# pierric/smart-chess-rust

Hardware: AMD Instinct MI355X
Metric: MCTS simulations/sec (whole node), self-play rollout=180, at 1/2/4/8 MI355X (higher is better)
Workload: dtype bf16

## Files before the change

smart-chess-rust_amd/csrc/nn_tower32.hpp:

```cpp
#pragma once
#include <type_traits>

#include "nn_kernels.hpp"

namespace scnn {

typedef __attribute__((ext_vector_type(16))) float f32x16;
typedef __attribute__((ext_vector_type(8))) int i32x8;

struct PrecBF16 {
    static constexpr bool FP8 = false;
    static constexpr int EB = 2;
    static constexpr int KS = 16;
    static constexpr int FB = 16;
    typedef bf16x8 frag;
};
struct PrecFP8 {
    static constexpr bool FP8 = true;
    static constexpr int EB = 1;
    static constexpr int KS = 64;
    static constexpr int FB = 32;
    typedef i32x8 frag;
};
template <class P>
// ... 109 lines not shown
    static_assert(TAPS % TPI == 0 && SPG % RS == 0 && PD < SPG, "bad ring / tap-group geometry");
    static_assert(SPG % AB == 0 && AD <= SPG, "bad image buffer geometry");
    const __amdgpu_buffer_rsrc_t rsrc = __builtin_amdgcn_make_buffer_rsrc(
        const_cast<bf16_t*>(Wp) + (size_t)wave_u * CT * (TB / 2), 0, 0x7fffffff, 0x00020000);
    const int voff = lane * 16;
    auto toffb = [](int t) { return (TAPS == 9) ? ((((t * 11) >> 5) - 1) * 10 + (t - 3 * ((t * 11) >> 5)) - 1) * PSB : 0; };
    frag xq[AB][2];
    int wcur = 0;
    int pc[TPI][2];
#pragma unroll
    for (int tl = 0; tl < TPI; tl++)
#pragma unroll
        for (int pt = 0; pt < 2; pt++) pc[tl][pt] = xoff + px[pt] + toffb(tl);
    if (!PRE) {
#pragma unroll
        for (int st = 0; st < PD; st++)
#pragma unroll
            for (int ct = 0; ct < CT; ct++) bq[st][ct] = wload_p<P>(rsrc, voff, ct, st * SBB);
    }
#pragma unroll
    for (int v = 0; v < AD; v++)
#pragma unroll
        for (int pt = 0; pt < 2; pt++) xq[v][pt] = lds_frag_p<P>(pc[v / KPT][pt] + (v % KPT) * KSB);
#pragma unroll 1
    for (int j = 0; j < NG; j++) {
        const int tn = (j + 1 == NG) ? 0 : j + 1;
        const int wnext = (j == NG - 1) ? next_first : tn * (SPG * SBB);
        int pn[TPI][2];
#pragma unroll
        for (int tl = 0; tl < TPI; tl++)
#pragma unroll
            for (int pt = 0; pt < 2; pt++) pn[tl][pt] = xoff + px[pt] + toffb(tn * TPI + tl);
#pragma unroll
        for (int u = 0; u < SPG; u++) {
            const int slot = u % RS;
#pragma unroll
            for (int ct = 0; ct < CT; ct++)
                bq[(slot + PD) % RS][ct] = (u + PD < SPG) ? wload_p<P>(rsrc, voff, ct, wcur + (u + PD) * SBB)
                                                          : wload_p<P>(rsrc, voff, ct, wnext + (u + PD - SPG) * SBB);
#pragma unroll
            for (int pt = 0; pt < 2; pt++) {
                const int v = u + AD;
                xq[v % AB][pt] = (v < SPG) ? lds_frag_p<P>(pc[v / KPT][pt] + (v % KPT) * KSB)
                                           : lds_frag_p<P>(pn[(v - SPG) / KPT][pt] + ((v - SPG) % KPT) * KSB);
            }
#pragma unroll
            for (int ct = 0; ct < CT; ct++)
#pragma unroll
                for (int pt = 0; pt < 2; pt++)
                    acc[ct][pt] = mma_p<P>(bq[slot][ct], xq[u % AB][pt], acc[ct][pt], sa[ct]);
#pragma unroll
            for (int m = 0; m < 2 * CT; m++) {
                __builtin_amdgcn_sched_group_barrier(0x008, 1, 0);
                if (P::FP8) {
                    __builtin_amdgcn_sched_group_barrier(0x100, CT == 1 ? 2 : 1, 0);
                    __builtin_amdgcn_sched_group_barrier(0x020, 1, 0);
                } else if (CT == 1) {
                    __builtin_amdgcn_sched_group_barrier(0x100, 1, 0);
                    if (m == 0) __builtin_amdgcn_sched_group_barrier(0x020, 1, 0);
                } else {
                    if ((m & 1) == 0)
                        __builtin_amdgcn_sched_group_barrier(0x100, 1, 0);
                    else
                        __builtin_amdgcn_sched_group_barrier(0x020, 1, 0);
                }
            }
            __builtin_amdgcn_sched_barrier(0);
        }
        wcur = wnext;
#pragma unroll
        for (int tl = 0; tl < TPI; tl++)
#pragma unroll
            for (int pt = 0; pt < 2; pt++) pc[tl][pt] = pn[tl][pt];
    }
}

struct LnStat {
    float rstd[2], nm[2];
};
template <int CT>
__device__ inline void ln_reduce(const f32x16 (&acc)[CT][2], LnStat& L, int count, int wave, int lane, float* s_stat2,
                                 int& parity, int& bad) {
    float2* st = reinterpret_cast<float2*>(s_stat2) + (parity & 1) * 256;
    parity ^= 1;
    const int i = lane & 31;
    float s[2], q[2];
#pragma unroll
    for (int pt = 0; pt < 2; pt++) {
        f32x2 a2 = {0.f, 0.f}, b2 = {0.f, 0.f};
#pragma unroll
        for (int ct = 0; ct < CT; ct++)
#pragma unroll
            for (int r = 0; r < 16; r += 2) {
                const f32x2 v = pair(acc[ct][pt], r);
                a2 += v;
                b2 = v * v + b2;
            }
        s[pt] = a2.x + a2.y;
        q[pt] = b2.x + b2.y;
    }
    {
        const auto rs = __builtin_amdgcn_permlane32_swap(__float_as_uint(s[0]), __float_as_uint(s[1]), false, false);
        const auto rq = __builtin_amdgcn_permlane32_swap(__float_as_uint(q[0]), __float_as_uint(q[1]), false, false);
        st[wave * 64 + lane] = make_float2(__uint_as_float(rs[0]) + __uint_as_float(rs[1]), __uint_as_float(rq[0]) + __uint_as_float(rq[1]));
    }
    __syncthreads();
    const float inv = 1.0f / (float)count;
#pragma unroll
    for (int pt = 0; pt < 2; pt++) {
        const int gp = pt * 32 + i;
        float2 a0 = st[gp], a1 = st[64 + gp], a2 = st[128 + gp], a3 = st[192 + gp];
        float S = (a0.x + a1.x) + (a2.x + a3.x);
        float Q = (a0.y + a1.y) + (a2.y + a3.y);
        float mean = S * inv;
        float var = Q * inv - mean * mean;
        bad |= (var != var) ? 1 : 0;
        var = fmaxf(var, 0.f);
        L.rstd[pt] = __frsqrt_rn(var + 1e-6f);
        L.nm[pt] = -mean * L.rstd[pt];
    }
}
template <int CT>
__device__ __forceinline__ void ln_apply(f32x16 (&acc)[CT][2], const LnStat& L, const ChP<CT>& G, const ChP<CT>& E, bool relu) {
#pragma unroll
    for (int pt = 0; pt < 2; pt++)
#pragma unroll
        for (int ct = 0; ct < CT; ct++)
#pragma unroll
            for (int r = 0; r < 16; r += 2) {
                const f32x2 t = pair(acc[ct][pt], r) * splat(L.rstd[pt]) + splat(L.nm[pt]);
                const f32x2 y = t * pair(G.v[ct][r >> 2], r & 3) + pair(E.v[ct][r >> 2], r & 3);
                acc[ct][pt][r] = relu ? fmaxf(y.x, 0.f) : y.x;
                acc[ct][pt][r + 1] = relu ? fmaxf(y.y, 0.f) : y.y;
            }
}
template <class P, int CT>
__device__ __forceinline__ void ln_apply_relu_store(const f32x16 (&acc)[CT][2], const LnStat& L, const ChP<CT>& G, const ChP<CT>& E,
                                                    const int (&pixbase)[2], int wave, int h) {
#pragma unroll
    for (int ct = 0; ct < CT; ct++)
#pragma unroll
        for (int pt = 0; pt < 2; pt++)
#pragma unroll
            for (int g = 0; g < 4; g++) {
                f32x2 y[2];
#pragma unroll
                for (int hf = 0; hf < 2; hf++) {
                    const f32x2 t = pair(acc[ct][pt], 4 * g + 2 * hf) * splat(L.rstd[pt]) + splat(L.nm[pt]);
                    y[hf] = t * pair(G.v[ct][g], 2 * hf) + pair(E.v[ct][g], 2 * hf);
                }
                store4<P, true>(pixbase[pt], chan32<CT>(wave, ct, g, h), y[0], y[1]);
            }
}
template <int CT>
__device__ inline void layernorm32(f32x16 (&acc)[CT][2], const ChP<CT>& G, const ChP<CT>& E, int count, bool relu, int wave,
                                   int lane, float* s_stat2, int& parity, int& bad) {
    LnStat L;
    ln_reduce<CT>(acc, L, count, wave, lane, s_stat2, parity, bad);
    ln_apply<CT>(acc, L, G, E, relu);
}

template <class P, int CT>
__device__ inline void store_image32(const f32x16 (&acc)[CT][2], const int (&pixbase)[2], int wave, int h) {
#pragma unroll
    for (int ct = 0; ct < CT; ct++)
#pragma unroll
        for (int pt = 0; pt < 2; pt++)
#pragma unroll
            for (int g = 0; g < 4; g++)
                store4<P, false>(pixbase[pt], chan32<CT>(wave, ct, g, h), pair(acc[ct][pt], 4 * g), pair(acc[ct][pt], 4 * g + 2));
}

template <int CTRL>
__device__ __forceinline__ float dpp_mov(float x) { return dpp_f<CTRL>(x); }
template <int LVL>
__device__ __forceinline__ float pool_xchg(float x) {
    if constexpr (LVL == 1) return dpp_mov<0x140>(x);
    else if constexpr (LVL == 2) return dpp_mov<0x141>(x);
    else if constexpr (LVL == 3) return dpp_mov<0x4E>(x);
    else return dpp_mov<0xB1>(x);
}
template <int NV, int W, int LVL>
__device__ __forceinline__ void pool_level(float (&v)[NV], int lane) {
    if constexpr (LVL < 5) {
        if constexpr (W >= 1) {
            if constexpr (LVL == 0) {
#pragma unroll
                for (int t = 0; t < W; t++) {
                    const auto r = __builtin_amdgcn_permlane16_swap(__float_as_uint(v[t]), __float_as_uint(v[t + W]), false, false);
                    v[t] = __uint_as_float(r[0]) + __uint_as_float(r[1]);
                }
            } else {
                const bool hi = (lane & (16 >> LVL)) != 0;
#pragma unroll
                for (int t = 0; t < W; t++) {
                    float send = hi ? v[t] : v[t + W], keep = hi ? v[t + W] : v[t];
                    v[t] = keep + pool_xchg<LVL>(send);
                }
            }
            pool_level<NV, W / 2, LVL + 1>(v, lane);
        } else {
            v[0] += pool_xchg<LVL>(v[0]);
            pool_level<NV, 0, LVL + 1>(v, lane);
        }
    }
}

template <class P, int CT, int TILES, int RS>
__device__ __forceinline__ void ring_fill(typename P::frag (&bq)[RS][CT], const bf16_t* __restrict__ Wp, int wave_u, int lane) {
    constexpr int TB = 64 * P::FB;
    const __amdgpu_buffer_rsrc_t rsrc = __builtin_amdgcn_make_buffer_rsrc(
        const_cast<bf16_t*>(Wp) + (size_t)wave_u * CT * (TB / 2), 0, 0x7fffffff, 0x00020000);
#pragma unroll
    for (int st = 0; st < RS - 1; st++)
#pragma unroll
        for (int ct = 0; ct < CT; ct++) bq[st][ct] = wload_p<P>(rsrc, lane * 16, ct, st * TILES * TB);
}
template <class P, int CT>
__device__ __forceinline__ void scale_load(int (&sa)[CT], const NetDev& net, int conv_idx, int wave, int lane) {
#pragma unroll
    for (int ct = 0; ct < CT; ct++)
        sa[ct] = P::FP8 ? __builtin_bit_cast(int, net.wf[net.f_scales + (size_t)((conv_idx * 8 + wave * CT + ct) * 64 + lane)]) : 127;
}

template <class P, int C>
struct TowerLds {
    static constexpr int IMG_BYTES = (100 * pix_stride<P>(C) > 4864 * 4) ? 100 * pix_stride<P>(C) : 4864 * 4;
    static constexpr int HIMG_BYTES = 64 * pix_stride<P>(HEAD);
    static constexpr int HIMG = IMG_BYTES;
    static constexpr int STAT = HIMG + HIMG_BYTES;
    static constexpr int VEC = STAT + 4096;
    static constexpr int SCL = VEC + 3072;
    static constexpr int RED = SCL + 1024;
    static constexpr int PAR = RED + 64;
    static constexpr int TOTAL = PAR + 15 * C * 2;
    static_assert(4864 * 4 <= IMG_BYTES, "policy logits (and the softmax pass that reads 19 x 256 of them) must fit in the image area");
    static_assert(IMG_BYTES % 16 == 0 && HIMG_BYTES % 16 == 0, "LDS regions must stay 16-byte aligned");
    static_assert(6 * HEAD * 4 + 3 * POL_PAD * 4 <= TOTAL - VEC, "head parameters must fit in the staging area");
};
static_assert(TowerLds<PrecBF16, 128>::TOTAL == 73088 && TowerLds<PrecBF16, 256>::TOTAL == 102528, "bf16 tower LDS");
static_assert(TowerLds<PrecFP8, 128>::TOTAL == 48960 && TowerLds<PrecFP8, 256>::TOTAL == 60544, "fp8 tower LDS");

struct NoPre {
    __device__ __forceinline__ bool operator()(int) const { return true; }
};
struct Fc1Hand {
    typedef __attribute__((ext_vector_type(4))) unsigned int u32x4;
    Fc1W w;
    uint32_t early;
    int have_a;
    u32x4 a[8];
};
struct NoHand {};
template <class P, int C, int RS, int TPI, int AB = SC_T32_AB, class Pre = NoPre, class Hand = NoHand>
__device__ __forceinline__ bool tower_body(const TowerArgs& A, const int pos, const int8_t* planes_lds, Pre pre, Hand& fhr) {
    constexpr bool FUSED = !std::is_same<Pre, NoPre>::value;
    constexpr bool HAND = std::is_same<Hand, Fc1Hand>::value;
    Hand* const fh = &fhr;
    typedef typename P::frag frag;
    constexpr int CT = C / 128;
    constexpr int TILES = C / 32;
    constexpr int PSB = pix_stride<P>(C);
    constexpr int HPSB = pix_stride<P>(HEAD);
    constexpr int EB = P::EB;
    constexpr int HRS = P::FP8 ? C / 64 : 8, HAB = P::FP8 ? 2 : SC_T32_AB;
    constexpr int H2RS = P::FP8 ? HEAD / 64 : 16, H2AB = P::FP8 ? 2 : SC_T32_AB;
    constexpr int NTW = C / 64;
    typedef TowerLds<P, C> Lds;
    unsigned char* smem = g_smem;
    float* s_stat = reinterpret_cast<float*>(smem + Lds::STAT);
    float* s_scl = reinterpret_cast<float*>(smem + Lds::SCL);
    float* s_red = reinterpret_cast<float*>(smem + Lds::RED);
    bf16_t* s_xb = reinterpret_cast<bf16_t*>(smem + Lds::VEC);
    float* s_z = reinterpret_cast<float*>(smem);

    const int tid = threadIdx.x, lane = tid & 63;
    const int wave = __builtin_amdgcn_readfirstlane(tid >> 6);
    const int i32 = lane & 31, h = lane >> 5;
    const NetDev& net = A.net;
    const int bp[2] = {gpix2board(0, i32), gpix2board(1, i32)};
    const int pixbase[2] = {hidx(bp[0]) * PSB, hidx(bp[1]) * PSB};
    const int px[2] = {pixbase[0] + h * P::FB, pixbase[1] + h * P::FB};

    frag ring[RS][CT];
    int sa[CT], san[CT];
    scale_load<P, CT>(sa, net, 0, wave, lane);
    scale_load<P, CT>(san, net, net.n_blocks > 0 ? 1 : 1 + 2 * net.n_blocks, wave, lane);
    ChP<CT> Bn;
    const int p_in = tid >> 2, q_in = tid & 3;
    uint32_t win[7];
    if (!FUSED && !planes_lds) {
        const uint32_t* src = reinterpret_cast<const uint32_t*>(A.boards + (size_t)pos * 7168 + p_in * 112 + q_in * 28);
#pragma unroll
        for (int k = 0; k < 7; k++) win[k] = src[k];
    }
    static_assert(C <= 256, "one parameter vector per thread");
    f32x4 spv = f32x4{0.f, 0.f, 0.f, 0.f};
    if (tid < 3 * C / 4) spv = *reinterpret_cast<const f32x4*>(net.wf + net.f_stem + tid * 4);
    else if (tid < C) spv = *reinterpret_cast<const f32x4*>(net.wf + net.f_blocks + (tid - 3 * C / 4) * 4);
    if (!FUSED || wave != 0) ring_fill<P, CT, TILES, RS>(ring, net.wb + net.o_stem, wave, lane);
    __builtin_amdgcn_sched_barrier(0);
    if constexpr (FUSED) {
        __shared__ int s_go;
        if (wave <= 1) {
            const bool go = pre(wave);
            if (wave == 0 && lane == 0) s_go = go ? 1 : 0;
            if (wave == 0) ring_fill<P, CT, TILES, RS>(ring, net.wb + net.o_stem, wave, lane);
        } else {
            uint4* z = reinterpret_cast<uint4*>(smem);
            for (int k = tid - 128; k < 100 * PSB / 16; k += 128) z[k] = make_uint4(0, 0, 0, 0);
        }
        __syncthreads();
        if (!s_go) return false;
    } else {
        uint4* z = reinterpret_cast<uint4*>(smem);
        for (int k = tid; k < 100 * PSB / 16; k += 256) z[k] = make_uint4(0, 0, 0, 0);
        __syncthreads();
    }
    if (FUSED || planes_lds) {
        const uint32_t* src = reinterpret_cast<const uint32_t*>(planes_lds + p_in * 112 + q_in * 28);
#pragma unroll
        for (int k = 0; k < 7; k++) win[k] = src[k];
    }
    {
        uint32_t* dst = reinterpret_cast<uint32_t*>(smem + hidx(p_in) * PSB + q_in * 28 * EB);
#pragma unroll
        for (int k = 0; k < 7; k++) {
            const uint32_t w = win[k];
            float v[4];
#pragma unroll
            for (int b = 0; b < 4; b++) v[b] = (float)(int8_t)((w >> (8 * b)) & 0xff);
            if constexpr (P::FP8) {
                dst[k] = pk_fp8x4(v[0], v[1], v[2], v[3]);
            } else {
                dst[2 * k] = pk_bf16(f32x2{v[0], v[1]});
                dst[2 * k + 1] = pk_bf16(f32x2{v[2], v[3]});
            }
        }
        if (tid < C) *reinterpret_cast<f32x4*>(g_smem + Lds::PAR + tid * 16) = spv;
    }
    __syncthreads();

    f32x16 acc[CT][2];
    int ln_parity = 0;
    int bad = 0;
    f32x16 res[CT][2];
    auto store_res = [&]() {
#pragma unroll
        for (int ct = 0; ct < CT; ct++)
#pragma unroll
            for (int pt = 0; pt < 2; pt++) res[ct][pt] = acc[ct][pt];
    };
    auto dump = [&](int stage) {
        if constexpr (FUSED) return;
        if (A.dbg && A.dbg_stage == stage) {
#pragma unroll
            for (int ct = 0; ct < CT; ct++)
#pragma unroll
                for (int pt = 0; pt < 2; pt++)
#pragma unroll
                    for (int r = 0; r < 16; r++)
                        A.dbg[((size_t)pos * 64 + bp[pt]) * C + chan32<CT>(wave, ct, r >> 2, h) + (r & 3)] = acc[ct][pt][r];
        }
    };

    {
        ch_load_lds<CT>(Bn, Lds::PAR, wave, h);
        acc_init<CT>(acc, Bn);
        const bf16_t* w0 = net.wb + net.o_stem;
        conv_mma32<P, 128, 9, CT, TILES, PSB, RS, TPI, true, AB>(0, w0, wave, lane, px, acc, ring, (int)((net.wb + net.o_blocks) - w0) * 2, sa);
        ChP<CT> G, E;
        ch_load_lds<CT>(G, Lds::PAR + C * 4, wave, h);
        ch_load_lds<CT>(E, Lds::PAR + 2 * C * 4, wave, h);
        ch_load_lds<CT>(Bn, Lds::PAR + 3 * C * 4, wave, h);
        layernorm32<CT>(acc, G, E, C, true, wave, lane, s_stat, ln_parity, bad);
    }
    store_res();
    store_image32<P, CT>(acc, pixbase, wave, h);
    __syncthreads();
    dump(0);
    const int head_conv0 = 1 + 2 * net.n_blocks;

#pragma unroll 1
    for (int b = 0; b < net.n_blocks; b++) {
        const bf16_t* wb = net.wb + net.o_blocks + (size_t)b * net.blk_stride_b;
        const float* wf = net.wf + net.f_blocks + (size_t)b * net.blk_stride_f;
        constexpr int NT1 = C / 32;
        constexpr int NTW1 = NT1 / 4;
        constexpr int PAR_V4 = 15 * C / 8;
        constexpr int NPV = (PAR_V4 + 255) / 256;
        constexpr int P_G1 = Lds::PAR, P_E1 = Lds::PAR + 4 * C, P_B2 = Lds::PAR + 8 * C, P_G2 = Lds::PAR + 12 * C, P_E2 = Lds::PAR + 16 * C;
        constexpr int P_SB1 = Lds::PAR + 20 * C, P_SB2 = Lds::PAR + 22 * C, P_BN = Lds::PAR + 26 * C;
        f32x4 pv[NPV];
#pragma unroll
        for (int k = 0; k < NPV; k++)
            if (tid + 256 * k < PAR_V4) pv[k] = *reinterpret_cast<const f32x4*>(wf + C + (size_t)(tid + 256 * k) * 4);
        __builtin_amdgcn_sched_barrier(0);
        acc_init<CT>(acc, Bn);
#pragma unroll
        for (int ct = 0; ct < CT; ct++) sa[ct] = san[ct];
        scale_load<P, CT>(san, net, 2 + 2 * b, wave, lane);
        conv_mma32<P, C, 9, CT, TILES, PSB, RS, TPI, true, AB>(0, wb, wave, lane, px, acc, ring, 9 * C * C * EB, sa);
#pragma unroll
        for (int k = 0; k < NPV; k++)
            if (tid + 256 * k < PAR_V4) *reinterpret_cast<f32x4*>(g_smem + Lds::PAR + (tid + 256 * k) * 16) = pv[k];
        {
            LnStat L;
            ln_reduce<CT>(acc, L, C, wave, lane, s_stat, ln_parity, bad);
            ChP<CT> G, E;
            ch_load_lds<CT>(G, P_G1, wave, h);
            ch_load_lds<CT>(E, P_E1, wave, h);
            ln_apply_relu_store<P, CT>(acc, L, G, E, pixbase, wave, h);
        }
        ch_load_lds<CT>(Bn, P_B2, wave, h);
        __syncthreads();
        acc_init<CT>(acc, Bn);
        {
            const int nxt = (b + 1 < net.n_blocks) ? (int)(net.blk_stride_b * 2 - (size_t)9 * C * C * EB) : 0;
#pragma unroll
            for (int ct = 0; ct < CT; ct++) sa[ct] = san[ct];
            scale_load<P, CT>(san, net, b + 1 < net.n_blocks ? 3 + 2 * b : head_conv0, wave, lane);
            conv_mma32<P, C, 9, CT, TILES, PSB, RS, TPI, true, AB>(0, wb + (size_t)9 * C * C * EB / 2, wave, lane, px, acc, ring, nxt, sa);
        }
        VecW<C, NTW1> w1;
        VecW<C / 2, NTW> w2;
        vec_w_load<C, NTW1, NT1>(w1, wb + (size_t)9 * C * C * EB, wave * NTW1, lane);
        vec_w_load<C / 2, NTW, C / 16>(w2, wb + (size_t)9 * C * C * EB + (size_t)C * (C / 2), wave * NTW, lane);
        __builtin_amdgcn_sched_barrier(0);
        {
            LnStat L;
            ln_reduce<CT>(acc, L, C, wave, lane, s_stat, ln_parity, bad);
            ChP<CT> G, E;
            ch_load_lds<CT>(G, P_G2, wave, h);
            ch_load_lds<CT>(E, P_E2, wave, h);
            ln_apply<CT>(acc, L, G, E, false);
        }
        {
            constexpr int NV = 16 * CT;
            float v[NV];
#pragma unroll
            for (int ct = 0; ct < CT; ct++)
#pragma unroll
                for (int r = 0; r < 16; r += 2) {
                    const f32x2 t = pair(acc[ct][0], r) + pair(acc[ct][1], r);
                    v[ct * 16 + r] = t.x;
                    v[ct * 16 + r + 1] = t.y;
                }
            pool_level<NV, NV / 2, 0>(v, lane);
            const int idx = (NV == 32) ? i32 : (i32 >> 1);
            s_xb[chan32<CT>(wave, idx >> 4, (idx & 15) >> 2, h) + (idx & 3)] = f2bf(v[0] * (1.0f / 64.0f));
        }
        float sb1[NTW1], sb2[NTW];
#pragma unroll
        for (int k = 0; k < NTW1; k++) sb1[k] = *reinterpret_cast<const float*>(g_smem + P_SB1 + (wave * (16 * NTW1) + (lane & 15) * NTW1 + k) * 4);
#pragma unroll
        for (int k = 0; k < NTW; k++) sb2[k] = *reinterpret_cast<const float*>(g_smem + P_SB2 + (chan0<NTW>(wave, lane) + k) * 4);
        __syncthreads();
        bf16_t* s_hid = s_xb + 256;
        {
            f32x4 hh[NTW1];
#pragma unroll
            for (int k = 0; k < NTW1; k++) hh[k] = f32x4{0.f, 0.f, 0.f, 0.f};
            vec_mma<C, NTW1>(s_xb, w1, lane, hh);
            if (lane < 16) {
#pragma unroll
                for (int k = 0; k < NTW1; k++) {
                    const int j = wave * (16 * NTW1) + (lane & 15) * NTW1 + k;
                    float t = hh[k][0] + sb1[k];
                    s_hid[j] = f2bf(fmaxf(t, 0.f));
                }
            }
        }
        __syncthreads();
        {
            f32x4 sc[NTW];
#pragma unroll
            for (int k = 0; k < NTW; k++) sc[k] = f32x4{0.f, 0.f, 0.f, 0.f};
            vec_mma<C / 2, NTW>(s_hid, w2, lane, sc);
            if (lane < 16) {
                const int c0 = chan0<NTW>(wave, lane);
#pragma unroll
                for (int k = 0; k < NTW; k++)
                    s_scl[c0 + k] = __builtin_amdgcn_rcpf(1.0f + __expf(-(sc[k][0] + sb2[k])));
            }
        }
#pragma unroll
        for (int ct = 0; ct < CT; ct++)
#pragma unroll
            for (int g = 0; g < 4; g++) {
                const int ch = chan32<CT>(wave, ct, g, h);
                const f32x4 sv = *reinterpret_cast<const f32x4*>(s_scl + ch);
#pragma unroll
                for (int pt = 0; pt < 2; pt++) {
                    const f32x4 rv = f32x4{res[ct][pt][4 * g], res[ct][pt][4 * g + 1], res[ct][pt][4 * g + 2], res[ct][pt][4 * g + 3]};
#pragma unroll
                    for (int k = 0; k < 4; k += 2) {
                        const f32x2 y = pair(acc[ct][pt], 4 * g + k) * pair(sv, k) + pair(rv, k);
                        acc[ct][pt][4 * g + k] = fmaxf(y.x, 0.f);
                        acc[ct][pt][4 * g + k + 1] = fmaxf(y.y, 0.f);
                    }
                }
            }
        store_res();
        store_image32<P, CT>(acc, pixbase, wave, h);
        ch_load_lds<CT>(Bn, P_BN, wave, h);
        __syncthreads();
        dump(b + 1);
    }
    dump(1000);

    const int gpb[2] = {i32 * HPSB, (32 + i32) * HPSB};
    constexpr int HP_V = Lds::VEC, HP_P1 = Lds::VEC + 3 * HEAD * 4, HP_P2 = Lds::VEC + 6 * HEAD * 4;
    f32x4 hpv[2];
#pragma unroll
    for (int k = 0; k < 2; k++)
        if (tid + 256 * k < 480) hpv[k] = *reinterpret_cast<const f32x4*>(net.wf + net.f_vhead + (size_t)(tid + 256 * k) * 4);
    __builtin_amdgcn_sched_barrier(0);
    frag hr[HRS][2];
    frag hr2[H2RS][1];
    int sh[2], sh2[1];
    scale_load<P, 2>(sh, net, head_conv0, wave, lane);
    {
        f32x16 hv[2][2];
#pragma unroll
        for (int ct = 0; ct < 2; ct++)
#pragma unroll
            for (int pt = 0; pt < 2; pt++)
#pragma unroll
                for (int r = 0; r < 16; r++) hv[ct][pt][r] = 0.f;
        conv_mma32<P, C, 1, 2, 8, PSB, HRS, 1, false, HAB>(0, net.wb + net.o_vconv, wave, lane, px, hv, hr,
                                                           (int)((net.wb + net.o_pconv1) - (net.wb + net.o_vconv)) * 2, sh);
        scale_load<P, 2>(sh, net, head_conv0 + 1, wave, lane);
        scale_load<P, 1>(sh2, net, head_conv0 + 2, wave, lane);
#pragma unroll
        for (int k = 0; k < 2; k++)
            if (tid + 256 * k < 480) *reinterpret_cast<f32x4*>(g_smem + Lds::VEC + (tid + 256 * k) * 16) = hpv[k];
        __builtin_amdgcn_sched_barrier(0);
        __syncthreads();
        ChP<2> Bv, G, E;
        ch_load_lds<2>(Bv, HP_V, wave, h);
#pragma unroll
        for (int ct = 0; ct < 2; ct++)
#pragma unroll
            for (int pt = 0; pt < 2; pt++)
#pragma unroll
                for (int r = 0; r < 16; r++) hv[ct][pt][r] += Bv.v[ct][r >> 2][r & 3];
        LnStat L;
        int badv = bad;
        ln_reduce<2>(hv, L, HEAD, wave, lane, s_stat, ln_parity, badv);
        ch_load_lds<2>(G, HP_V + HEAD * 4, wave, h);
        ch_load_lds<2>(E, HP_V + 2 * HEAD * 4, wave, h);
        ln_apply<2>(hv, L, G, E, true);
        const __amdgpu_buffer_rsrc_t hrs = __builtin_amdgcn_make_buffer_rsrc(A.hval + (size_t)pos * (64 * HEAD), 0, 0x7fffffff, 0x00020000);
        const bool wt = HAND && A.fc1_arrive;
#pragma unroll
        for (int ct = 0; ct < 2; ct++)
#pragma unroll
            for (int pt = 0; pt < 2; pt++) {
                const int off = (((wave * 2 + ct) * 2 + pt) * 64 + lane) * 32;
#pragma unroll
                for (int q = 0; q < 2; q++) {
                    typedef __attribute__((ext_vector_type(4))) unsigned int u32x4;
                    u32x4 v = {pk_bf16(pair(hv[ct][pt], 8 * q)), pk_bf16(pair(hv[ct][pt], 8 * q + 2)), pk_bf16(pair(hv[ct][pt], 8 * q + 4)),
                               pk_bf16(pair(hv[ct][pt], 8 * q + 6))};
                    if (badv) v = u32x4{0x7fc07fc0u, 0x7fc07fc0u, 0x7fc07fc0u, 0x7fc07fc0u};
                    if (wt) __builtin_amdgcn_raw_buffer_store_b128(v, hrs, off + 16 * q, 0, AUX_SC1);
                    else __builtin_amdgcn_raw_buffer_store_b128(v, hrs, off + 16 * q, 0, 0);
                }
            }
    }
    {
        ChP<2> Bv, G, E;
        ch_load_lds<2>(Bv, HP_P1, wave, h);
        f32x16 hp[2][2];
        acc_init<2>(hp, Bv);
        conv_mma32<P, C, 1, 2, 8, PSB, HRS, 1, true, HAB>(0, net.wb + net.o_pconv1, wave, lane, px, hp, hr, 0, sh);
        if (HAND && A.fc1_arrive) asm volatile("s_waitcnt vmcnt(0)" ::: "memory");
        ring_fill<P, 1, 4, H2RS>(hr2, net.wb + net.o_pconv2, wave, lane);
        __builtin_amdgcn_sched_barrier(0);
        LnStat L;
        ln_reduce<2>(hp, L, HEAD, wave, lane, s_stat, ln_parity, bad);
        if (HAND && A.fc1_arrive && tid == 0)
            __hip_atomic_fetch_add(A.fc1_arrive + (pos >> 6) * 32, 1u, __ATOMIC_RELAXED, __HIP_MEMORY_SCOPE_AGENT);
        ch_load_lds<2>(G, HP_P1 + HEAD * 4, wave, h);
        ch_load_lds<2>(E, HP_P1 + 2 * HEAD * 4, wave, h);
        ln_apply<2>(hp, L, G, E, false);
        const int xb[2] = {Lds::HIMG + gpb[0], Lds::HIMG + gpb[1]};
        store_image32<P, 2>(hp, xb, wave, h);
    }
    __syncthreads();
    {
        ChP<1> Bv, G, E;
        ch_load_lds<1>(Bv, HP_P2, wave, h);
        f32x16 z[1][2];
        acc_init<1>(z, Bv);
        const int pxh[2] = {gpb[0] + h * P::FB, gpb[1] + h * P::FB};
        conv_mma32<P, HEAD, 1, 1, 4, HPSB, H2RS, 1, true, H2AB>(Lds::HIMG, net.wb + net.o_pconv2, wave, lane, pxh, z, hr2, 0, sh2);
        uint32_t first = 0;
        if (HAND && A.fc1_arrive && tid == 0 && !A.fc1_acquire)
            first = __hip_atomic_load(A.fc1_arrive + (pos >> 6) * 32, __ATOMIC_RELAXED, __HIP_MEMORY_SCOPE_AGENT);
        LnStat L;
        ln_reduce<1>(z, L, 73, wave, lane, s_stat, ln_parity, bad);
        ch_load_lds<1>(G, HP_P2 + POL_PAD * 4, wave, h);
        ch_load_lds<1>(E, HP_P2 + 2 * POL_PAD * 4, wave, h);
        ln_apply<1>(z, L, G, E, false);
        __syncthreads();
#pragma unroll
        for (int pt = 0; pt < 2; pt++)
#pragma unroll
            for (int r = 0; r < 16; r++) {
                const int ch = chan32<1>(wave, 0, r >> 2, h) + (r & 3);
                if (ch < 73) s_z[ch * 64 + bp[pt]] = z[0][pt][r];
            }
// ... 59 lines not shown
```

smart-chess-rust_amd/csrc/search_select.hpp:

```cpp
#pragma once
#include <type_traits>
#include <hip/hip_runtime.h>

#include "mcts_types.hpp"
#include "position_chain.hpp"

namespace sc {

using scw::dpp_i, scw::wave_sum_fixed, scw::wave_sum_i;

__device__ __forceinline__ int wave_argmax_last(float u, int idx) {
    unsigned b = __builtin_bit_cast(unsigned, u + 0.0f);
    unsigned key = (b & 0x80000000u) ? ~b : (b | 0x80000000u);
    int hi = idx >= 0 ? (int)key : 0, lo = idx;
    auto step = [&](int ohi, int olo) {
        const bool take = olo >= 0 && (lo < 0 || (unsigned)ohi > (unsigned)hi || ((unsigned)ohi == (unsigned)hi && olo > lo));
        hi = take ? ohi : hi;
        lo = take ? olo : lo;
    };
    step(dpp_i<0xB1>(hi), dpp_i<0xB1>(lo));
    step(dpp_i<0x4E>(hi), dpp_i<0x4E>(lo));
    step(dpp_i<0x141>(hi), dpp_i<0x141>(lo));
    step(dpp_i<0x140>(hi), dpp_i<0x140>(lo));
    int bh = __builtin_amdgcn_readlane(hi, 0), bl = __builtin_amdgcn_readlane(lo, 0);
#pragma unroll
    for (int r = 16; r < 64; r += 16) {
        const int oh = __builtin_amdgcn_readlane(hi, r), ol = __builtin_amdgcn_readlane(lo, r);
        const bool take = ol >= 0 && (bl < 0 || (unsigned)oh > (unsigned)bh || ((unsigned)oh == (unsigned)bh && ol > bl));
        bh = take ? oh : bh;
        bl = take ? ol : bl;
    }
    return bl;
}
__device__ __forceinline__ int wave_argmax_last_lane(float u, bool has) {
    unsigned b = __builtin_bit_cast(unsigned, u + 0.0f);
    unsigned key = (b & 0x80000000u) ? ~b : (b | 0x80000000u);
    int k = has ? (int)key : 0;
    auto umax = [](int a, int b2) { return (int)((unsigned)a > (unsigned)b2 ? (unsigned)a : (unsigned)b2); };
    int m = k;
    m = umax(m, dpp_i<0xB1>(m));
    m = umax(m, dpp_i<0x4E>(m));
    m = umax(m, dpp_i<0x141>(m));
    m = umax(m, dpp_i<0x140>(m));
    const int wm = umax(umax(__builtin_amdgcn_readlane(m, 0), __builtin_amdgcn_readlane(m, 16)),
                        umax(__builtin_amdgcn_readlane(m, 32), __builtin_amdgcn_readlane(m, 48)));
    const unsigned long long mask = __ballot(has && k == wm);
    return mask ? 63 - __clzll((long long)mask) : -1;
}
__device__ __forceinline__ NodeHdr uniform(const NodeHdr& q) {
    NodeHdr r;
    r.fc = uniform(q.fc);
    r.nc = (uint16_t)uniform((int)q.nc);
    r.ps = (uint16_t)uniform((int)q.ps);
    return r;
}
__device__ __forceinline__ GameCtl uniform(const GameCtl& q) {
    GameCtl r;
    r.status = uniform(q.status);
    r.ply = uniform(q.ply);
    r.sim = uniform(q.sim);
    r.n_nodes = uniform(q.n_nodes);
    r.n_exp = uniform(q.n_exp);
    r.leaf = uniform(q.leaf);
    r.path_len = uniform(q.path_len);
    r.leaf_kind = uniform(q.leaf_kind);
    r.n_legal = uniform(q.n_legal);
    r.leaf_value = __builtin_bit_cast(float, uniform(__builtin_bit_cast(int, q.leaf_value)));
    r.err = (uint32_t)uniform((int)q.err);
    r.trace_slot = uniform(q.trace_slot);
    r.game_id = uniform((bb_t)q.game_id);
    r.start_ply = uniform(q.start_ply);
    r.rollout_cur = uniform(q.rollout_cur);
    return r;
}

__device__ inline float u01_open(uint64_t& st) {
#pragma clang fp contract(off)
    st = mix64(st);
    return ((float)(st >> 40) + 0.5f) * (1.0f / 16777216.0f);
}
__device__ inline float gamma03(uint64_t st) {
#pragma clang fp contract(off)
    const float LN2 = 0.69314718f;
    const float alpha = 0.3f;
    const float boost = __builtin_amdgcn_exp2f(__builtin_amdgcn_logf(u01_open(st)) * (1.0f / alpha));
    const float d = alpha + 1.0f - 1.0f / 3.0f;
    const float c = 0.3390317518f;
    for (int it = 0; it < 64; it++) {
        float a = u01_open(st), b = u01_open(st);
        float x = __builtin_amdgcn_sqrtf(-2.0f * LN2 * __builtin_amdgcn_logf(a)) * __builtin_amdgcn_cosf(b);
        float v = 1.0f + c * x;
        if (v <= 0.0f) continue;
        v = v * v * v;
        float u = u01_open(st);
        if (LN2 * __builtin_amdgcn_logf(u) < 0.5f * x * x + d - d * v + d * (LN2 * __builtin_amdgcn_logf(v))) return boost * d * v;
    }
    return boost * d;
}

constexpr int DEPTH_LDS = 1024;

#define SC_STAMP(k)                                                                       \
    do {                                                                                  \
        if constexpr (SC_ST) {                                                            \
            if (p.dbg_cycles && lane == 0) p.dbg_cycles[(size_t)g * 32 + (k)] = clock64(); \
        }                                                                                 \
    } while (0)

struct HelperBox {
    int state, idx, root_ply, pad;
};
__device__ __forceinline__ void helper_post(HelperBox* box, int lane, int state, int idx, int root_ply) {
    if (!box) return;
    if (lane == 0) {
        box->idx = idx;
        box->root_ply = root_ply;
    }
    wave_sync();
    if (lane == 0) *reinterpret_cast<volatile int*>(&box->state) = state;
}
__device__ __forceinline__ void dev_encode_helper(const SpParams& p, int g, int lane, HelperBox* box, int8_t* s_stage, Position* s_leaf_p,
                                                  uint16_t* s_ps, Position* s_hist) {
    int st = 0;
    for (int spin = 0; spin < (1 << 22) && st == 0; spin++) {
        st = *reinterpret_cast<volatile int*>(&box->state);
        if (st == 0) __builtin_amdgcn_s_sleep(2);
    }
    st = __builtin_amdgcn_readfirstlane(st);
    if (st == 0 && lane == 0) atomicOr(&p.cnt->err, ERR_HELPER_TIMEOUT);
    if (st != 1 && st != 3) return;
    wave_sync();
    const int idx = __builtin_amdgcn_readfirstlane(box->idx), root_ply = __builtin_amdgcn_readfirstlane(box->root_ply);
    DevChain ch{p.hist + (size_t)g * p.hist_cap, root_ply, p.tpos + (size_t)g * p.tpos_cap, s_ps, s_leaf_p, idx};
    if (st == 3) {
        const bb_t key0 = s_leaf_p->key;
        const uint8_t rf = (uint8_t)__builtin_amdgcn_readfirstlane((int)rep_flags_wave(ch, idx, key0, lane));
        const uint8_t fl = (uint8_t)((s_leaf_p->flags & F_IRREV) | rf);
        wave_sync();
        if (lane == 0) {
            s_leaf_p->flags = fl;
            box->pad = fl;
        }
        wave_sync();
        if (lane == 0) *reinterpret_cast<volatile int*>(&box->state) = 4;
    }
    stage_history(ch, idx, lane, s_hist);
    wave_sync();
    encode_wave(s_hist, idx < 7 ? idx + 1 : 8, lane, s_stage, nullptr, p.meta + (size_t)g * 8);
}

template <bool PLANES_TO_HBM = true, bool SC_ST = true>
__device__ __forceinline__ bool dev_select(const SpParams& p, int g, int lane, int8_t* s_stage, move_t* s_moves, Position* s_leaf_p,
                                        uint16_t* s_ps, Position* s_hist, const GameCtl& cs_pre, bool cs_pre_valid,
                                        HelperBox* box = nullptr) {
#pragma clang fp contract(off)
    Position& s_leaf = *s_leaf_p;
    SC_STAMP(2);
    GameCtl& c = p.ctl[g];
    GameCtl cs = cs_pre;
    if (!cs_pre_valid) cs = uniform(c);
    const Position root_raw = p.tpos[(size_t)g * p.tpos_cap];
    const NodeHdr hdr_raw = p.H[(size_t)g * p.node_cap];
    const size_t nb0 = (size_t)g * p.node_cap + (1 + lane < p.node_cap ? 1 + lane : p.node_cap - 1);
    const int pf_n = p.N[nb0];
    const float pf_w = p.W[nb0], pf_p = p.P[nb0];
    const NodeHdr pf_h = p.H[nb0];
    __builtin_amdgcn_sched_barrier(0);
    const Position root = uniform(root_raw);
    NodeHdr hdr = uniform(hdr_raw);
    if (cs.status != ST_ACTIVE) {
        if (lane == 0) c.leaf_kind = LK_NONE;
        helper_post(box, lane, 2, 0, 0);
        return false;
    }
    const size_t nb = (size_t)g * p.node_cap;
    const int32_t* N = p.N + nb;
    const float* W = p.W + nb;
    const float* P = p.P + nb;
    float* U = p.U + nb;
    const uint16_t* MV = p.MV + nb;
    const NodeHdr* H = p.H + nb;
    int32_t* path = p.path + (size_t)g * p.max_depth;
    const Position* hist = p.hist + (size_t)g * p.hist_cap;
    Position* tpos = p.tpos + (size_t)g * p.tpos_cap;
    const int root_ply = cs.ply;
    const int root_turn = root.turn;
    const int dmax = p.max_depth < DEPTH_LDS ? p.max_depth : DEPTH_LDS;

    int node = 0, depth = 0, parent_ps = 0;
    if (lane == 0) {
        path[0] = 0;
        s_ps[0] = 0;
    }
    uint32_t err = 0;
    for (;;) {
        const int nc = hdr.nc;
        if (nc == 0) break;
        const int fc = hdr.fc;
        const int nr = (nc + 63) >> 6;
        int best_i = 0;
        NodeHdr nxt;
        auto level = [&](auto nrc) {
#pragma clang fp contract(off)
            constexpr int NRM = decltype(nrc)::value;
            int cn[NRM];
            float cw[NRM], cp[NRM];
            NodeHdr ch_[NRM];
#pragma unroll
            for (int r = 0; r < NRM; r++) {
                cn[r] = 0;
                cw[r] = 0.f;
                cp[r] = 0.f;
                ch_[r] = NodeHdr{-1, 0, 0};
                if (r < nr) {
                    int i = lane + 64 * r;
                    bool ok = i < nc;
                    if (r == 0 && depth == 0 && fc == 1) {
                        cn[0] = ok ? pf_n : 0;
                        cw[0] = ok ? pf_w : 0.f;
                        cp[0] = ok ? pf_p : 0.f;
                        ch_[0] = ok ? pf_h : NodeHdr{-1, 0, 0};
                    } else {
                        cn[r] = ok ? N[fc + i] : 0;
                        cw[r] = ok ? W[fc + i] : 0.f;
                        cp[r] = ok ? P[fc + i] : 0.f;
                        ch_[r] = ok ? H[fc + i] : NodeHdr{-1, 0, 0};
                    }
                }
            }
            if (nc > 1) {
                const bool reverse_q = ((root_turn ^ (depth & 1)) == BLACK);
                const bool noisy = depth == 0 && p.with_noise;
                float* nz = p.noise + (size_t)g * MAXC;
                float nzv[NRM];
#pragma unroll
                for (int r = 0; r < NRM; r++) nzv[r] = 0.f;
                if (noisy) {
                    if (!p.external_noise) {
                        float gsum = 0.0f;
#pragma unroll
                        for (int r = 0; r < NRM; r++) {
                            int i = lane + 64 * r;
                            if (i < nc) {
                                nzv[r] = gamma03(sc_rng(p.seed, cs.game_id, (uint64_t)root_ply, 3, (uint64_t)cs.sim * 256 + (uint64_t)i));
                                gsum += nzv[r];
                            }
                        }
                        gsum = wave_sum_fixed(gsum);
#pragma unroll
                        for (int r = 0; r < NRM; r++) {
                            int i = lane + 64 * r;
                            nzv[r] = nzv[r] / gsum;
                            if (i < nc) nz[i] = nzv[r];
                        }
                    } else {
#pragma unroll
                        for (int r = 0; r < NRM; r++) {
                            int i = lane + 64 * r;
                            if (i < nc) nzv[r] = nz[i];
                        }
                    }
                }
                int tot = 0;
#pragma unroll
                for (int r = 0; r < NRM; r++) tot += cn[r];
                tot = wave_sum_i(tot);
                const float sqrt_total = sqrtf((float)tot);
                float best_u = 0.0f;
                best_i = -1;
#pragma unroll
                for (int r = 0; r < NRM; r++) {
                    int i = lane + 64 * r;
                    if (r < nr && i < nc) {
                        float prior = cp[r];
                        if (noisy) prior = prior * (1.0f - p.epsilon) + nzv[r] * p.epsilon;
                        float average_award = cw[r] / ((float)cn[r] + 1e-4f) * (reverse_q ? -1.0f : 1.0f);
                        float exploration = (sqrt_total + 0.01f) / (1.0f + (float)cn[r]) * p.cpuct * prior;
                        float u = average_award + exploration;
                        U[fc + i] = u;
                        if (!isfinite(u)) err |= ERR_NONFINITE_UCT;
                        if (best_i < 0 || u >= best_u) {
                            best_u = u;
                            best_i = i;
                        }
                    }
                }
                if constexpr (NRM == 1) best_i = wave_argmax_last_lane(best_u, best_i >= 0);
                else best_i = wave_argmax_last(best_u, best_i);
            }
            best_i = __builtin_amdgcn_readfirstlane(best_i);
            const int rr = best_i >> 6;
            NodeHdr mine = ch_[0];
#pragma unroll
            for (int r = 1; r < NRM; r++)
                if (rr == r) mine = ch_[r];
            nxt.fc = __builtin_amdgcn_readlane(mine.fc, best_i & 63);
            int packed = __builtin_amdgcn_readlane((int)mine.nc | ((int)mine.ps << 16), best_i & 63);
            nxt.nc = (uint16_t)(packed & 0xffff);
            nxt.ps = (uint16_t)((unsigned)packed >> 16);
        };
        if (nr == 1) level(std::integral_constant<int, 1>{});
        else level(std::integral_constant<int, 4>{});
        parent_ps = hdr.ps;
        node = fc + best_i;
        hdr = nxt;
        depth++;
        if (depth >= dmax) {
            err |= ERR_DEPTH_OVERFLOW;
            depth--;
            break;
        }
        if (lane == 0) {
            path[depth] = node;
            s_ps[depth] = hdr.ps;
        }
    }
    SC_STAMP(3);
    if (p.dbg_cycles && lane == 0) p.dbg_cycles[(size_t)g * 32 + 7] = depth;
    unsigned long long anyerr = __ballot(err != 0);
    if (anyerr) {
        for (int o = 32; o > 0; o >>= 1) err |= __shfl_xor(err, o, 64);
        if (lane == 0) {
            c.err = cs.err | err;
            atomicOr(&p.cnt->err, (int)err);
        }
    }
    const int fcl = hdr.fc;
    if (lane == 0) {
        c.leaf = node;
        c.path_len = depth + 1;
    }
    if (fcl <= -2) {
        if (lane == 0) {
            c.leaf_kind = LK_TERM_CACHED;
            c.leaf_value = fcl == -2 ? 0.0f : fcl == -3 ? 1.0f : -1.0f;
            c.n_legal = 0;
        }
        helper_post(box, lane, 2, 0, 0);
        return false;
    }
    Position pos;
    if (depth == 0) {
        pos = root;
    } else {
        pos = uniform(tpos[parent_ps]);
        make_move(pos, (move_t)__builtin_amdgcn_readfirstlane((int)MV[node]));
    }
    if (lane == 0) s_leaf = pos;
    wave_sync();
    DevChain ch{hist, root_ply, tpos, s_ps, &s_leaf, root_ply + depth};
    const bool rep_by_helper = box && depth > 0;
    if (depth > 0 && !box) {
        uint8_t rf = (uint8_t)__builtin_amdgcn_readfirstlane((int)rep_flags_wave(ch, root_ply + depth, pos.key, lane));
        pos.flags = (uint8_t)((pos.flags & F_IRREV) | rf);
        wave_sync();
        if (lane == 0) s_leaf.flags = pos.flags;
        wave_sync();
    }
    SC_STAMP(4);
    if (box) helper_post(box, lane, rep_by_helper ? 3 : 1, root_ply + depth, root_ply);
    else stage_history(ch, root_ply + depth, lane, s_hist);
    if (lane == 0 && !rep_by_helper) tpos[cs.n_exp] = pos;
    int n = 0;
    bool in_check = gen_legal_wave(pos, s_moves, lane, n);
    wave_sync();
    SC_STAMP(5);
    if (depth == 0 && p.rollout_factor > 0.f && lane == 0) {
        const int r = (int)((float)n * p.rollout_factor);
        c.rollout_cur = r < 300 ? r : 300;
    }
    if (n == 0) {
        if (lane == 0) {
            c.leaf_kind = LK_TERM_NEW;
            c.leaf_value = in_check ? (pos.turn == WHITE ? -1.0f : 1.0f) : 0.0f;
            c.n_legal = 0;
        }
        return false;
    }
    uint16_t* lm = p.legal_mv + (size_t)g * MAXC;
    uint16_t* li = p.legal_idx + (size_t)g * MAXC;
    uint32_t bad = 0;
    for (int i = lane; i < n; i += 64) {
        move_t m = s_moves[i];
        int idx = move_index(m, pos.turn);
        if (idx < 0) {
            bad = 1;
            idx = 0;
        }
        lm[i] = m;
        li[i] = (uint16_t)idx;
    }
    if (__ballot(bad) && lane == 0) {
        c.err = cs.err | err | ERR_BAD_MOVE_INDEX;
        atomicOr(&p.cnt->err, ERR_BAD_MOVE_INDEX);
    }
    if (rep_by_helper) {
        int st = 3;
        for (int spin = 0; spin < (1 << 22) && st != 4; spin++) {
            st = *reinterpret_cast<volatile int*>(&box->state);
            if (st != 4) __builtin_amdgcn_s_sleep(1);
        }
        st = __builtin_amdgcn_readfirstlane(st);
        wave_sync();
        if (st != 4 && lane == 0) atomicOr(&p.cnt->err, ERR_HELPER_TIMEOUT);
        pos.flags = (uint8_t)__builtin_amdgcn_readfirstlane(box->pad);
        if (lane == 0) tpos[cs.n_exp] = pos;
    }
    const int idx = root_ply + depth;
    if (!box) encode_wave(s_hist, idx < 7 ? idx + 1 : 8, lane, s_stage, PLANES_TO_HBM ? p.boards + (size_t)g * 7168 : nullptr, p.meta + (size_t)g * 8);
    if (lane == 0) {
        c.leaf_kind = LK_EVAL;
        c.n_legal = n;
        p.n_legal[g] = n;
    }
    SC_STAMP(6);
    return true;
}

}
```

smart-chess-rust_amd/csrc/step_kernels.hip:

```cpp
#include "search_expand.hpp"
#include "nn_kernels.hpp"
#include "nn_tower32.hpp"

#include "launchers.hpp"
#include "tower_config.hpp"

namespace scstep {

__device__ __forceinline__ void fc1_tail(const scnn::TowerArgs& A, const sc::SpParams& p, const int g, const bool ran, scnn::Fc1Hand& fh) {
    const int tid = threadIdx.x, lane = tid & 63;
    const int wave = __builtin_amdgcn_readfirstlane(tid >> 6);
    const int mb = g >> 6, ks = g & 63;
    uint32_t* ctr = A.fc1_arrive + mb * 32;
    if (!ran) {
        if (tid == 0) __hip_atomic_fetch_add(ctr, 1u, __ATOMIC_RELAXED, __HIP_MEMORY_SCOPE_AGENT);
        scnn::fc1_wload(fh.w, A.net, ks, 64, wave, lane);
        __builtin_amdgcn_sched_barrier(0);
    }
    const scnn::Fc1W& w = fh.w;
    const bool have_a = ran && fh.have_a;
    if (tid == 0 && !have_a) {
        const uint64_t t0 = __builtin_amdgcn_s_memrealtime();
        uint32_t seen = ran ? fh.early : __hip_atomic_load(ctr, __ATOMIC_RELAXED, __HIP_MEMORY_SCOPE_AGENT);
        while ((int32_t)(seen - A.fc1_target) < 0) {
            __builtin_amdgcn_s_sleep(4);
            const uint64_t waited = __builtin_amdgcn_s_memrealtime() - t0;
            if (waited > 20000000ull) {
                atomicOr(&p.cnt->err, sc::ERR_HANDOFF_TIMEOUT);
                break;
            }
            if (waited > 100000ull && (__hip_atomic_load(&p.cnt->err, __ATOMIC_RELAXED, __HIP_MEMORY_SCOPE_AGENT) & sc::ERR_HANDOFF_TIMEOUT)) break;
            seen = __hip_atomic_load(ctr, __ATOMIC_RELAXED, __HIP_MEMORY_SCOPE_AGENT);
        }
        if (A.fc1_acquire) __builtin_amdgcn_fence(__ATOMIC_ACQUIRE, "agent");
        asm volatile("s_waitcnt vmcnt(0)" ::: "memory");
    }
    __syncthreads();
    scnn::bf16_t* s_a = reinterpret_cast<scnn::bf16_t*>(scnn::g_smem);
    if (!have_a) scnn::fc1_load_a(fh.a, A.hval, mb, ks, tid);
    scnn::fc1_put_a(s_a, fh.a, tid);
    __syncthreads();
    scnn::fc1_mma_store(w, s_a, A.vpart, A.n_pos, mb, ks, 64, wave, lane);
}

template <class P, int C, int RS, int TPI, int AB, bool STAMPS = false>
__global__ __launch_bounds__(256, 1) void k_step(scnn::TowerArgs A, sc::SpParams p, int do_expand) {
    __shared__ __attribute__((aligned(16))) int8_t s_stage[7168];
    __shared__ sc::move_t s_moves[sc::MAXC];
    __shared__ sc::Position s_pos;
    __shared__ sc::Position s_hist[8];
    __shared__ uint16_t s_ps[sc::DEPTH_LDS];
    __shared__ sc::HelperBox s_box;
    const int g = blockIdx.x;
    const int lane = threadIdx.x & 63;
    scnn::kernarg_prefetch<sizeof(scnn::TowerArgs) + sizeof(sc::SpParams) + sizeof(int)>();
#define PHASE_STAMP(k, cond) do { if constexpr (STAMPS) { if (p.dbg_cycles && (cond)) p.dbg_cycles[(size_t)g * 32 + (k)] = __builtin_amdgcn_s_memrealtime(); } } while (0)
    PHASE_STAMP(24, threadIdx.x == 0);
    if (threadIdx.x == 0) s_box.state = 0;
    __syncthreads();
    auto search = [&](int wave) -> bool {
        if (wave == 1) {
            sc::dev_encode_helper(p, g, lane, &s_box, s_stage, &s_pos, s_ps, s_hist);
            return true;
        }
        constexpr bool SC_ST = STAMPS;
        SC_STAMP(0);
        sc::GameCtl cs_pre{};
        bool cs_pre_valid = false;
        if (do_expand) {
            sc::dev_expand<SC_ST>(p, g, lane, &s_pos, cs_pre, cs_pre_valid);
            __builtin_amdgcn_wave_barrier();
        }
        SC_STAMP(1);
        const bool need_net = sc::dev_select<false, SC_ST>(p, g, lane, s_stage, s_moves, &s_pos, s_ps, s_hist, cs_pre, cs_pre_valid, &s_box);
        PHASE_STAMP(25, lane == 0);
        return need_net;
    };
    scnn::Fc1Hand fh;
    const bool ran = scnn::tower_body<P, C, RS, TPI, AB>(A, g, s_stage, search, fh);
    PHASE_STAMP(26, threadIdx.x == 0);
    if (A.fc1_arrive) fc1_tail(A, p, g, ran, fh);
    PHASE_STAMP(27, threadIdx.x == 0);
#undef PHASE_STAMP
}

}

namespace scl {
template <class T, bool STAMPS = false>
constexpr auto step_kernel(T) { return &scstep::k_step<typename T::P, T::C, T::RS, T::TPI, T::AB, STAMPS>; }

const char* step_init() {
    for (bool fp8 : {false, true})
        for (int C : {128, 256}) {
            const hipError_t e = scnn::with_tower_cfg(fp8, C, [](auto cfg) {
                return hipFuncSetAttribute(reinterpret_cast<const void*>(step_kernel(cfg)), hipFuncAttributeMaxDynamicSharedMemorySize, cfg.LDS_BYTES);
            });
            if (e != hipSuccess) return hipGetErrorString(e);
        }
    const hipError_t e = hipFuncSetAttribute(reinterpret_cast<const void*>(step_kernel<scnn::TowerBf16N, true>({})), hipFuncAttributeMaxDynamicSharedMemorySize,
                                             scnn::TowerBf16N::LDS_BYTES);
    return e == hipSuccess ? nullptr : hipGetErrorString(e);
}
int step_blocks_per_cu(const scnn::NetLayout& net) {
    int n = 0;
    const hipError_t e = scnn::with_tower_cfg(net.fp8, net.C, [&](auto cfg) {
        return hipOccupancyMaxActiveBlocksPerMultiprocessor(&n, step_kernel(cfg), 256, cfg.LDS_BYTES);
    });
    return e == hipSuccess && n > 0 ? n : 1;
}
void step(const scnn::TowerArgs& a, const sc::SpParams& p, int do_expand, hipStream_t s) {
    const dim3 grid(p.n_slots), block(256);
    if (!a.net.fp8 && a.net.C == 128 && p.dbg_cycles)
        hipLaunchKernelGGL((step_kernel<scnn::TowerBf16N, true>({})), grid, block, scnn::TowerBf16N::LDS_BYTES, s, a, p, do_expand);
    else
        scnn::with_tower_cfg(a.net.fp8, a.net.C, [&](auto cfg) { hipLaunchKernelGGL(step_kernel(cfg), grid, block, cfg.LDS_BYTES, s, a, p, do_expand); });
}
}
```

Before: 2.184 million.

## Precompute Dirichlet gamma noise on a helper wave in parallel with expand/select

Wave 2 now speculatively predicts the game's sim counter and computes per-lane gamma noise samples into LDS while wave 0 runs expand and select. At the root the selecting wave spin-waits for the staged samples and, if game id, ply and sim match, uses them instead of computing gamma03 itself. This takes the RNG/gamma work off wave 0's serial critical path. The cost is an extra LDS handshake, a possible spin-wait, and a fallback recompute when the prediction misses. The tower's fused pre-phase is also reordered so every wave calls pre().

```diff
diff --git a/smart-chess-rust_amd/csrc/nn_tower32.hpp b/smart-chess-rust_amd/csrc/nn_tower32.hpp
--- a/smart-chess-rust_amd/csrc/nn_tower32.hpp
+++ b/smart-chess-rust_amd/csrc/nn_tower32.hpp
@@ -435,13 +435,14 @@
     __builtin_amdgcn_sched_barrier(0);
     if constexpr (FUSED) {
         __shared__ int s_go;
-        if (wave <= 1) {
-            const bool go = pre(wave);
-            if (wave == 0 && lane == 0) s_go = go ? 1 : 0;
-            if (wave == 0) ring_fill<P, CT, TILES, RS>(ring, net.wb + net.o_stem, wave, lane);
-        } else {
+        if (wave >= 2) {
             uint4* z = reinterpret_cast<uint4*>(smem);
             for (int k = tid - 128; k < 100 * PSB / 16; k += 128) z[k] = make_uint4(0, 0, 0, 0);
+        }
+        const bool go = pre(wave);
+        if (wave == 0) {
+            if (lane == 0) s_go = go ? 1 : 0;
+            ring_fill<P, CT, TILES, RS>(ring, net.wb + net.o_stem, wave, lane);
         }
         __syncthreads();
         if (!s_go) return false;
diff --git a/smart-chess-rust_amd/csrc/search_select.hpp b/smart-chess-rust_amd/csrc/search_select.hpp
--- a/smart-chess-rust_amd/csrc/search_select.hpp
+++ b/smart-chess-rust_amd/csrc/search_select.hpp
@@ -149,13 +149,51 @@
     encode_wave(s_hist, idx < 7 ? idx + 1 : 8, lane, s_stage, nullptr, p.meta + (size_t)g * 8);
 }
 
-template <bool PLANES_TO_HBM = true, bool SC_ST = true>
+struct NoiseBox {
+    uint64_t game_id;
+    int ply, sim, state;
+};
+__device__ __forceinline__ void dev_noise_helper(const SpParams& p, int g, int lane, bool expanding, NoiseBox* nbox, float* gam) {
+    if (!p.with_noise || p.external_noise) return;
+    const GameCtl craw = p.ctl[g];
+    const int status = uniform(craw.status), leaf_kind = uniform(craw.leaf_kind), ply = uniform(craw.ply);
+    const uint64_t game_id = uniform((bb_t)craw.game_id);
+    const int sim = uniform(craw.sim) + (expanding && status == ST_ACTIVE && leaf_kind != LK_NONE ? 1 : 0);
+    gam[lane] = gamma03(sc_rng(p.seed, game_id, (uint64_t)ply, 3, (uint64_t)sim * 256 + (uint64_t)lane));
+    if (lane == 0) {
+        nbox->game_id = game_id;
+        nbox->ply = ply;
+        nbox->sim = sim;
+    }
+    wave_sync();
+    if (lane == 0) *reinterpret_cast<volatile int*>(&nbox->state) = 1;
+}
+__device__ __forceinline__ bool noise_take(NoiseBox* nbox, const float* gam, uint64_t game_id, int ply, int sim, int lane, int nc, float& out) {
+    int st = 0;
+    for (int spin = 0; spin < (1 << 22) && st == 0; spin++) {
+        st = *reinterpret_cast<volatile int*>(&nbox->state);
+        if (st == 0) __builtin_amdgcn_s_sleep(1);
+    }
+    st = __builtin_amdgcn_readfirstlane(st);
+    if (st == 0) return false;
+    wave_sync();
+    const bool hit = uniform((bb_t)nbox->game_id) == game_id && __builtin_amdgcn_readfirstlane(nbox->ply) == ply &&
+                     __builtin_amdgcn_readfirstlane(nbox->sim) == sim;
+    if (!hit) return false;
+    out = lane < nc ? gam[lane] : 0.f;
+    return true;
+}
+
+template <bool PLANES_TO_HBM = true, bool SC_ST = true, bool NOISE_AHEAD = false>
 __device__ __forceinline__ bool dev_select(const SpParams& p, int g, int lane, int8_t* s_stage, move_t* s_moves, Position* s_leaf_p,
                                         uint16_t* s_ps, Position* s_hist, const GameCtl& cs_pre, bool cs_pre_valid,
-                                        HelperBox* box = nullptr) {
+                                        HelperBox* box = nullptr, NoiseBox* nbox = nullptr, const float* gam = nullptr) {
 #pragma clang fp contract(off)
     Position& s_leaf = *s_leaf_p;
     SC_STAMP(2);
+    if constexpr (SC_ST && NOISE_AHEAD) {
+        if (p.dbg_cycles && lane == 0) p.dbg_cycles[(size_t)g * 32 + 8] = 0;
+    }
     GameCtl& c = p.ctl[g];
     GameCtl cs = cs_pre;
     if (!cs_pre_valid) cs = uniform(c);
@@ -238,12 +276,22 @@
                 if (noisy) {
                     if (!p.external_noise) {
                         float gsum = 0.0f;
-#pragma unroll
-                        for (int r = 0; r < NRM; r++) {
-                            int i = lane + 64 * r;
-                            if (i < nc) {
-                                nzv[r] = gamma03(sc_rng(p.seed, cs.game_id, (uint64_t)root_ply, 3, (uint64_t)cs.sim * 256 + (uint64_t)i));
-                                gsum += nzv[r];
+                        if constexpr (NOISE_AHEAD && NRM == 1) {
+                            const bool staged = noise_take(nbox, gam, cs.game_id, root_ply, cs.sim, lane, nc, nzv[0]);
+                            if constexpr (SC_ST) {
+                                if (p.dbg_cycles && lane == 0) p.dbg_cycles[(size_t)g * 32 + 8] = staged ? 2 : 1;
+                            }
+                            if (!staged && lane < nc)
+                                nzv[0] = gamma03(sc_rng(p.seed, cs.game_id, (uint64_t)root_ply, 3, (uint64_t)cs.sim * 256 + (uint64_t)lane));
+                            if (lane < nc) gsum += nzv[0];
+                        } else {
+#pragma unroll
+                            for (int r = 0; r < NRM; r++) {
+                                int i = lane + 64 * r;
+                                if (i < nc) {
+                                    nzv[r] = gamma03(sc_rng(p.seed, cs.game_id, (uint64_t)root_ply, 3, (uint64_t)cs.sim * 256 + (uint64_t)i));
+                                    gsum += nzv[r];
+                                }
                             }
                         }
                         gsum = wave_sum_fixed(gsum);
diff --git a/smart-chess-rust_amd/csrc/step_kernels.hip b/smart-chess-rust_amd/csrc/step_kernels.hip
--- a/smart-chess-rust_amd/csrc/step_kernels.hip
+++ b/smart-chess-rust_amd/csrc/step_kernels.hip
@@ -51,16 +51,25 @@
     __shared__ sc::Position s_hist[8];
     __shared__ uint16_t s_ps[sc::DEPTH_LDS];
     __shared__ sc::HelperBox s_box;
+    __shared__ sc::NoiseBox s_nbox;
+    __shared__ float s_gam[64];
     const int g = blockIdx.x;
     const int lane = threadIdx.x & 63;
     scnn::kernarg_prefetch<sizeof(scnn::TowerArgs) + sizeof(sc::SpParams) + sizeof(int)>();
 #define PHASE_STAMP(k, cond) do { if constexpr (STAMPS) { if (p.dbg_cycles && (cond)) p.dbg_cycles[(size_t)g * 32 + (k)] = __builtin_amdgcn_s_memrealtime(); } } while (0)
     PHASE_STAMP(24, threadIdx.x == 0);
-    if (threadIdx.x == 0) s_box.state = 0;
+    if (threadIdx.x == 0) {
+        s_box.state = 0;
+        s_nbox.state = 0;
+    }
     __syncthreads();
     auto search = [&](int wave) -> bool {
         if (wave == 1) {
             sc::dev_encode_helper(p, g, lane, &s_box, s_stage, &s_pos, s_ps, s_hist);
+            return true;
+        }
+        if (wave >= 2) {
+            if (wave == 2) sc::dev_noise_helper(p, g, lane, do_expand != 0, &s_nbox, s_gam);
             return true;
         }
         constexpr bool SC_ST = STAMPS;
@@ -72,7 +81,7 @@
             __builtin_amdgcn_wave_barrier();
         }
         SC_STAMP(1);
-        const bool need_net = sc::dev_select<false, SC_ST>(p, g, lane, s_stage, s_moves, &s_pos, s_ps, s_hist, cs_pre, cs_pre_valid, &s_box);
+        const bool need_net = sc::dev_select<false, SC_ST, true>(p, g, lane, s_stage, s_moves, &s_pos, s_ps, s_hist, cs_pre, cs_pre_valid, &s_box, &s_nbox, s_gam);
         PHASE_STAMP(25, lane == 0);
         return need_net;
     };
```

Measured after the change: 2.171 million. No clear change (-0.6%).
